# sail-sg/finetune-fair-diffusion

Measured on AMD Instinct MI355X. Metric: training-images/sec (SD-v1.5 512^2, 20-step DPM-Solver++ unroll, fairness-finetune step), higher is better.
Workload: dtype f16

## Files before the change

finetune_fair_diffusion_amd/ops.py:

```python
import ctypes
import os
import math

import torch

from . import lib as _lib

ACT = dict(none=0, silu=1, quick_gelu=2, gelu=3, relu=4, hardswish=5, hardsigmoid=6, geglu=7)
CONV_NORMAL, CONV_STRIDE2, CONV_UP2, CONV_TRANS2 = 0, 1, 2, 3
F16, F32 = _lib.torch_working_dtype(), torch.float32


def _stream():
    return ctypes.c_void_p(torch.cuda.current_stream().cuda_stream)


def _p(t):
    if t is None:
        return None
    assert t.is_cuda, "fairdiff ops need device tensors (no CPU path)"
    return ctypes.c_void_p(t.data_ptr())


DELAY = None
# ... 164 lines not shown
    d.alpha, d.M, d.N, d.K, d.batch = 1.0, rows, N, K, Z
    d.sA, d.sB, d.sC = a_view.stride(0), 0, rows * N
    _gemm_call(d, False)
    return out


def conv3x3(x, w, B, H, W, *, mode=CONV_NORMAL, bias=None, rowbias=None, residual=None, act="none", out=None, gn_stats=False):
    Cin = x.shape[1]
    Cout = w.shape[0]
    assert w.shape[1] == 9 * Cin and x.shape[0] == B * H * W
    _chk(x), _chk(w)
    if mode == CONV_NORMAL:
        Ho, Wo = H, W
    elif mode == CONV_STRIDE2:
        Ho, Wo = (H + 1) // 2, (W + 1) // 2
    else:
        Ho, Wo = 2 * H, 2 * W
    M = B * Ho * Wo
    if out is None:
        out = torch.empty((M, Cout), dtype=F16, device=x.device)
    d = _lib.GemmDesc()
    d.A, d.lda, d.B, d.ldb, d.C, d.ldc = x.data_ptr(), Cin, w.data_ptr(), 9 * Cin, out.data_ptr(), out.stride(0)
    if bias is not None:
        d.bias = _chk(bias, F32).data_ptr()
    if rowbias is not None:
        d.rowbias, d.ld_rowbias, d.rows_per_batch = _chk(rowbias).data_ptr(), rowbias.stride(0), (M if rowbias.shape[0] == 1 else Ho * Wo)
    if residual is not None:
        d.residual, d.ldr = _chk(residual).data_ptr(), residual.stride(0)
    d.alpha, d.M, d.N, d.K, d.act, d.batch = 1.0, M, Cout, 9 * Cin, ACT[act], 1
    d.out_dtype = 1 if out.dtype == F32 else 0
    d.conv, d.conv_mode, d.Bn, d.H, d.W, d.Cin, d.Ho, d.Wo = 1, mode, B, H, W, Cin, Ho, Wo
    _gemm_call(d, True, out, gn_stats)
    return out, Ho, Wo


CONV_UP2P, CONV_UP2P_BWD, CONV_UP2PI = 4, 5, 6
_BIG_TILES = (256320, 128320, 128160, 256128, 256256, 512128)
_NO_UP2P = os.environ.get("FD_NO_UP2P") is not None


def _up2p_desc(x, w, out, B, H, W, Cin, Cout, bwd, bias=None):
    d = _lib.GemmDesc()
    if bwd:
        d.K, d.conv_mode, d.H, d.W = 16 * Cin, CONV_UP2P_BWD, 2 * H, 2 * W
    else:
        d.K, d.conv_mode, d.H, d.W = 4 * Cin, CONV_UP2PI, H, W
    d.A, d.lda, d.B, d.ldb, d.C, d.ldc = x.data_ptr(), Cin, w.data_ptr(), d.K, out.data_ptr(), Cout
    if bias is not None:
        d.bias = _chk(bias, F32).data_ptr()
    d.alpha, d.M, d.N, d.act, d.batch, d.out_dtype = 1.0, B * H * W, Cout, ACT["none"], 1, 0
    d.conv, d.Bn, d.Cin, d.Ho, d.Wo = 1, B, Cin, H, W
    ws = gemm_workspace()
    d.workspace, d.workspace_bytes = ws.data_ptr(), ws.numel() * 4
    return d


def conv_up2(x, conv, B, H, W):
    Cin, Cout = conv.cin, conv.cout
    if not _NO_UP2P and Cin % 64 == 0 and Cout % 8 == 0:
        out = torch.empty((4 * B * H * W, Cout), dtype=F16, device=x.device)
        d = _up2p_desc(_chk(x), conv.wk_up2p, out, B, H, W, Cin, Cout, False, conv.bias)
        if _lib.get().fd_gemm_tile(ctypes.byref(d)) in _BIG_TILES:
            _gemm_call(d, True, out, gn_stats=(H * W) % 32 == 0)
            if getattr(out, "gn_stats", None) is not None:
                out.gn_stats = out.gn_stats + ((H * W) // 32,)
            return out, 2 * H, 2 * W
    return conv3x3(x, conv.wk, B, H, W, mode=CONV_UP2, bias=conv.bias)


def conv_up2_bwd(dy, conv, B, H, W):
    Cin, Cout = conv.cin, conv.cout
    if not _NO_UP2P and Cout % 64 == 0 and Cin % 8 == 0:
        out = torch.empty((B * H * W, Cin), dtype=F16, device=dy.device)
        d = _up2p_desc(_chk(dy), conv.wd_up2p, out, B, H, W, Cout, Cin, True)
        if _lib.get().fd_gemm_tile(ctypes.byref(d)) % 1000000 in _BIG_TILES:
            _gemm_call(d, True)
            return out
    dxu, _, _ = conv3x3(dy, conv.wd, B, 2 * H, 2 * W)
    return downsum2x2(dxu, B, H, W, Cin)


def conv_small_cin(x, w, bias, B, H, W, Cin, Cout, k, stride=1, nchw=True, act="none"):
    pad = (k - 1) // 2
    Ho, Wo = (H + 2 * pad - k) // stride + 1, (W + 2 * pad - k) // stride + 1
    y = torch.empty((B * Ho * Wo, Cout), dtype=F16, device=x.device)
    assert x.is_contiguous() and x.dtype in (F16, F32)
    _call("fd_conv_small_cin", _p(x), int(x.dtype == F32), int(nchw), _p(_chk(w, F32)), _p(bias), _p(y), B, H, W, Cin, Cout, k, stride,
          ACT[act], _stream())
    return y, Ho, Wo


def conv_small_cin_bwd(dy, w, B, H, W, Cin, Cout, k, stride=1, scale=1.0):
    dx = torch.empty((B, Cin, H, W), dtype=F32, device=dy.device)
    _call("fd_conv_small_cin_bwd", _p(_chk(dy)), _p(_chk(w, F32)), _p(dx), B, H, W, Cin, Cout, k, stride, scale, _stream())
    return dx


def nhwc_to_nchw(x, B, HW, C, *, out_dtype=F32, scale=1.0, lo=-math.inf, hi=math.inf):
    y = torch.empty((B, C, HW), dtype=out_dtype, device=x.device)
    _call("fd_nhwc_to_nchw", _p(x), x.stride(0), _p(y), int(out_dtype == F32), B, HW, C, scale, lo, hi, _stream())
    return y


def clamp_bwd(pre, dimg, B, HW, C, lo=-1.0, hi=1.0):
    out = torch.empty_like(dimg)
    _call("fd_clamp_bwd", _p(pre), pre.stride(0), _p(_chk(dimg, F32)), _p(out), B, HW, C, lo, hi, _stream())
    return out


_scratch = {}


def scratch(nfloats, device):
    key = (device.index if device.index is not None else torch.cuda.current_device(), torch.cuda.current_stream().cuda_stream)
    t = _scratch.get(key)
    if t is None or t.numel() < nfloats:
        t = torch.empty(max(nfloats, 1 << 22), dtype=F32, device=device)
        _scratch[key] = t
    return t


def groupnorm(x1, x2, B, HW, groups, eps, gamma, beta, silu):
    C1, C2 = x1.shape[1], (x2.shape[1] if x2 is not None else 0)
    st = torch.empty((B, groups, 2), dtype=F32, device=x1.device)
    y = torch.empty((B * HW, C1 + C2), dtype=F16, device=x1.device)
    s1, s2 = getattr(x1, "gn_stats", None), (getattr(x2, "gn_stats", None) if x2 is not None else None)
    if (s1 is not None and (x2 is None or s2 is not None) and HW % s1[1] == 0 and (s2 is None or HW % s2[1] == 0)
            and ((C1 + C2) // groups) % 10 == 0 and s1[0].shape[0] * s1[1] == B * HW and (s2 is None or s2[0].shape[0] * s2[1] == B * HW)):
        per1 = s1[2] if len(s1) > 2 else 0
        per2 = s2[2] if (s2 is not None and len(s2) > 2) else 0
        _call("fd_groupnorm_fwd_stats_p", _p(_chk(x1)), C1, _p(x2), C2, B, HW, groups, eps, _p(gamma), _p(beta), int(silu), _p(y), _p(st),
              _p(s1[0]), s1[1], per1, _p(s2[0]) if s2 is not None else None, s2[1] if s2 is not None else 0, per2, _stream())
        return y, st
    sc = scratch(B * 64 * groups * 2, x1.device)
    _call("fd_groupnorm_fwd", _p(_chk(x1)), C1, _p(x2), C2, B, HW, groups, eps, _p(gamma), _p(beta), int(silu), _p(y), _p(st), _p(sc), _stream())
    return y, st


def groupnorm_bwd(x1, x2, dy, B, HW, groups, stats, gamma, beta, silu, add1=None, add2=None, need_dx2=True):
    C1, C2 = x1.shape[1], (x2.shape[1] if x2 is not None else 0)
    dx1 = torch.empty_like(x1)
    dx2 = torch.empty_like(x2) if (x2 is not None and need_dx2) else None
    sc = scratch(B * 65 * groups * 2, x1.device)
    _call("fd_groupnorm_bwd", _p(x1), C1, _p(x2), C2, _p(_chk(dy)), B, HW, groups, _p(stats), _p(gamma), _p(beta), int(silu), _p(sc),
          _p(add1), _p(add2), _p(dx1), _p(dx2), _stream())
    return dx1, dx2


def geglu_bwd_interleaved(proj_il, dy):
    M, F2 = proj_il.shape
    d = torch.empty_like(proj_il)
    _call("fd_geglu_bwd_interleaved", _p(_chk(proj_il)), _p(_chk(dy)), _p(d), M, F2 // 2, _stream())
    return d


def layernorm(x, gamma, beta, eps=1e-5, save_stats=False):
    M, C = x.shape
    y = torch.empty_like(x)
    st = torch.empty((M, 2), dtype=F32, device=x.device) if save_stats else None
    _call("fd_layernorm_fwd", _p(_chk(x)), _p(gamma), _p(beta), _p(y), _p(st), M, C, eps, _stream())
    return (y, st) if save_stats else y


def layernorm_bwd(x, dy, gamma, stats, add=None):
    M, C = x.shape
    dx = torch.empty_like(x)
    _call("fd_layernorm_bwd", _p(_chk(x)), _p(_chk(dy)), _p(gamma), _p(stats), _p(add), _p(dx), M, C, _stream())
    return dx


def geglu(proj):
    M, F2 = proj.shape
    y = torch.empty((M, F2 // 2), dtype=F16, device=proj.device)
    _call("fd_geglu_fwd", _p(_chk(proj)), _p(y), M, F2 // 2, _stream())
    return y


def geglu_bwd(proj, dy):
    M, F2 = proj.shape
    d = torch.empty_like(proj)
    _call("fd_geglu_bwd", _p(proj), _p(_chk(dy)), _p(d), M, F2 // 2, _stream())
    return d


def act_fwd(x, act):
    y = torch.empty_like(x)
    _call("fd_act_fwd", _p(_chk(x)), _p(y), x.numel(), ACT[act], _stream())
    return y


def act_bwd(z, dy, act):
    dx = torch.empty_like(z)
    _call("fd_act_bwd", _p(_chk(z)), _p(_chk(dy)), _p(dx), z.numel(), ACT[act], _stream())
    return dx


def add(a, b, sa=1.0, sb=1.0, out=None):
    if out is None:
        out = torch.empty_like(a)
    _call("fd_add", _p(_chk(a)), _p(b), _p(out), a.numel(), sa, sb, _stream())
    return out


def copy_cols(src, dst, cols):
    _call("fd_copy_cols", _p(src), src.stride(0), _p(dst), dst.stride(0), src.shape[0], cols, _stream())


def _rows(t):
    assert t.dtype == F16 and t.dim() == 2 and t.stride(1) == 1, (t.dtype, t.shape, t.stride())
    return t.stride(0)


def transpose_btc(x, B, T, C, Tp=None, out=None):
    Tp = Tp or ((T + 7) // 8 * 8)
    y = torch.empty((B, C, Tp), dtype=F16, device=x.device) if out is None else out
    assert y.shape == (B, C, Tp) and y.dtype == F16 and y.is_contiguous()
    _call("fd_transpose_btc", _p(x), _rows(x), _p(y), B, T, C, Tp, _stream())
    return y


def downsum2x2(x, B, H, W, C):
    y = torch.empty((B * H * W, C), dtype=F16, device=x.device)
    _call("fd_downsum2x2", _p(_chk(x)), _p(y), B, H, W, C, _stream())
    return y


def softmax_rows(x, scale=1.0, mask=None, mask_t=0, mask_ht=0):
    rows, cols = x.numel() // x.shape[-1], x.shape[-1]
    y = torch.empty_like(x)
    _call("fd_softmax_rows", _p(_chk(x)), _p(y), rows, cols, scale, _p(mask), mask_t, mask_ht, _stream())
    return y


def softmax_rows_bwd(p, dp, scale=1.0):
    rows, cols = p.numel() // p.shape[-1], p.shape[-1]
    ds = torch.empty_like(p)
    _call("fd_softmax_rows_bwd", _p(_chk(p)), _p(_chk(dp)), _p(ds), rows, cols, scale, _stream())
    return ds


def to_f16(x, scale=1.0):
    y = torch.empty(x.shape, dtype=F16, device=x.device)
    _call("fd_cast_f32_to_f16", _p(_chk(x, F32)), _p(y), x.numel(), scale, _stream())
    return y


def to_f32(x, scale=1.0):
    y = torch.empty(x.shape, dtype=F32, device=x.device)
    _call("fd_cast_f16_to_f32", _p(_chk(x)), _p(y), x.numel(), scale, _stream())
    return y


LOG2E = 1.4426950408889634
PRESCALED_Q = os.environ.get("FD_NO_PRESCALED_Q") is None


def q_prescale(d):
    return (d ** -0.5) * LOG2E if (PRESCALED_Q and d % 16 == 8) else None


def attn_fwd(q, k, v, B, H, Tq, Tk, d, kv_div=1, scale=None, need_lse=False, kv_rows=None, prescaled=False):
    Tkr = kv_rows or Tk
    assert _rows(v) == _rows(k) and v.shape == k.shape
    o = torch.empty((q.shape[0], H * d), dtype=F16, device=q.device)
    lse = torch.empty((B, H, Tq), dtype=F32, device=q.device) if need_lse else None
    scale = scale if scale is not None else d ** -0.5
    _call("fd_attn_fwd", _p(q), _p(k), _p(v), _p(o), _p(lse), B, H, Tq, Tk, Tkr, d, kv_div,
          -scale if prescaled else scale, _rows(q), _rows(k), _stream())
    return (o, lse) if need_lse else o


def attn_bwd(q, k, v, o, do, lse, B, H, Tq, Tk, d, kv_div=1, scale=None, dk_acc=None, dv_acc=None, kv_rows=None, dqkv=None,
             dk_out=None, dv_out=None, prescaled=False):
    scale = scale if scale is not None else d ** -0.5
    if prescaled:
        scale = -scale
    Tkr = kv_rows or Tk
    C = H * d
    assert _rows(k) == _rows(v)
    Dd = torch.empty((B, H, Tq), dtype=F32, device=q.device)
    if dqkv is not None:
        assert kv_div == 1 and dqkv.shape == (q.shape[0], 3 * C) and dqkv.is_contiguous() and Tkr == Tk and dqkv.dtype == F16
        dq, dk, dv = dqkv[:, :C], dqkv[:, C:2 * C], dqkv[:, 2 * C:]
        lddkv = 3 * C
    else:
        dq = torch.empty((q.shape[0], C), dtype=F16, device=q.device)
        lddkv = C
        if dk_out is not None:
            assert dk_out.dtype == F32 and dv_out.dtype == F32 and dk_out.shape == (k.shape[0], C) and dv_out.shape == dk_out.shape and Tkr == Tk
            assert dk_out.is_contiguous() and dv_out.is_contiguous() and B % kv_div == 0
            slabs = torch.empty((2, kv_div) + tuple(dk_out.shape), dtype=F32, device=q.device)
            dk, dv = slabs[0], slabs[1]
        elif dk_acc is not None:
            dk, dv = dk_acc, dv_acc
            assert dk.dtype == F32 and dv.dtype == F32 and dk.shape == (k.shape[0], C) and Tkr == Tk
        else:
            assert kv_div == 1, "shared K/V (kv_div > 1) needs the fp32 accumulators dk_acc / dv_acc"
            mk = torch.empty if Tkr == Tk else torch.zeros
            dk, dv = mk((k.shape[0], C), dtype=F16, device=q.device), mk((k.shape[0], C), dtype=F16, device=q.device)
    _call("fd_attn_bwd_dq", _p(q), _p(k), _p(v), _p(_chk(do)), _p(lse), _p(Dd), _p(_chk(o)), _p(dq), B, H, Tq, Tk, Tkr, d,
          kv_div, scale, _rows(q), _rows(k), _rows(dq), _stream())
    _call("fd_attn_bwd_dkdv", _p(q), _p(k), _p(v), _p(do), _p(lse), _p(Dd), _p(dk), _p(dv), B, H, Tq, Tk, Tkr, d, kv_div, scale,
          _rows(q), _rows(k), lddkv, 2 if dk_out is not None else int(dk_acc is not None), _stream())
    if dk_out is not None:
        n = dk_out.numel()
        _call("fd_sum_slabs", _p(dk), _p(dk_out), kv_div, n, _stream())
# ... 259 lines not shown
```

finetune_fair_diffusion_amd/unet.py:

```python
import math

import torch

from . import ops
from .layers import (F16, F32, Conv3x3, Linear, LoRAPair, Norm, ParamBank, ResnetBlock, lora_linear_bwd, lora_linear_fwd)
from .weights import UNetConfig, unet_attn_names, unet_lora_param_shapes, unet_param_shapes


BWD_SLOT = [None]


class _Out:
    def __init__(self, sample):
        self.sample = sample


class LoRAAttnProcessor:

    def __init__(self, hidden_size, cross_attention_dim=None, rank=4):
        self.hidden_size, self.cross_attention_dim, self.rank = hidden_size, cross_attention_dim, rank

    def to(self, *a, **k):
        return self

# ... 1 lines not shown
class AttnLoRA:

    def __init__(self, bank, name):
        self.q, self.k, self.v, self.out = (LoRAPair(bank, f"{name}.{p}_lora.down.weight", f"{name}.{p}_lora.up.weight")
                                            for p in ("to_q", "to_k", "to_v", "to_out"))
        dev = bank.flat.device
        rp = self.q.rp
        if self.q.K == self.k.K:
            C = self.q.N
            self.down_qkv16 = torch.zeros((3 * rp, C), dtype=F16, device=dev)
            self.down_qkvT16 = torch.zeros((C, 3 * rp), dtype=F16, device=dev)
            self.up_qkv16 = torch.zeros((3 * C, 3 * rp), dtype=F16, device=dev)
            self.upT_qkv16 = torch.zeros((3 * rp, 3 * C), dtype=F16, device=dev)
            for i, p in enumerate((self.q, self.k, self.v)):
                p.place(self.down_qkv16[i * rp:(i + 1) * rp], self.down_qkvT16[:, i * rp:(i + 1) * rp],
                        self.up_qkv16[i * C:(i + 1) * C, i * rp:(i + 1) * rp], self.upT_qkv16[i * rp:(i + 1) * rp, i * C:(i + 1) * C])
            self.down_kv16 = self.down_qkv16[rp:]
        else:
            self.down_kv16 = torch.zeros((2 * rp, self.k.K), dtype=F16, device=dev)
            self.q.place()
            self.k.place(down16=self.down_kv16[:rp])
            self.v.place(down16=self.down_kv16[rp:])
        self.out.place()

    def pairs(self):
        return (self.q, self.k, self.v, self.out)

    def refresh(self):
        from .layers import refresh_pairs
        refresh_pairs(self.pairs())


class TransformerBlock:

    def __init__(self, sd, p, dev, C, heads, groups, xdim):
        self.C, self.heads, self.d, self.groups, self.xdim = C, heads, C // heads, groups, xdim
        self.p = p
        self.norm = Norm(sd, p + "norm", dev)
        self.proj_in = Linear(sd, p + "proj_in", dev, conv1x1=True)
        self.proj_out = Linear(sd, p + "proj_out", dev, conv1x1=True)
        b = p + "transformer_blocks.0."
        self.ln1, self.ln2, self.ln3 = Norm(sd, b + "norm1", dev), Norm(sd, b + "norm2", dev), Norm(sd, b + "norm3", dev)
        self.q1, self.k1, self.v1, self.o1 = (Linear(sd, b + "attn1." + n, dev) for n in ("to_q", "to_k", "to_v", "to_out.0"))
        assert self.q1.bias is None and self.k1.bias is None and self.v1.bias is None
        self.wqkv = torch.cat([self.q1.w, self.k1.w, self.v1.w], 0).contiguous()
        self._wqkvT = None
        self.q2, self.k2, self.v2, self.o2 = (Linear(sd, b + "attn2." + n, dev) for n in ("to_q", "to_k", "to_v", "to_out.0"))
        ff1, self.ff2 = Linear(sd, b + "ff.net.0.proj", dev), Linear(sd, b + "ff.net.2", dev)
        self.ff1_wi, self.ff1_bi = ops.interleave_geglu(ff1.w, ff1.bias)
        self._ff1_wiT = None
        self.lora1 = self.lora2 = None
        self.name1, self.name2 = b + "attn1.processor", b + "attn2.processor"
        self.cross = None
        self.lean = False

    def prepare_cross(self, enc, Bk, L, record, static=False):
        lo = self.lora2
        te = ops.gemm(enc, lo.down_kv16) if lo is not None else None
        rp = lo.k.rp if lo is not None else 0
        old = None
        if lo is not None:
            K = ops.gemm(enc, self.k2.w, a2=te[:, :rp], b2=lo.k.up16)
            V = ops.gemm(enc, self.v2.w, a2=te[:, rp:], b2=lo.v.up16)
        elif static:
            old = self.cross if (self.cross is not None and self.cross.get("static") and self.cross["K"].shape == (Bk * L, self.C)) else None
            K = ops.gemm(enc, self.k2.w, out=old["K"] if old else None)
            V = ops.gemm(enc, self.v2.w, out=old["V"] if old else None)
            if old is None:
                self.static_generation = getattr(self, "static_generation", 0) + 1
        else:
            K, V = ops.gemm(enc, self.k2.w), ops.gemm(enc, self.v2.w)
        self.cross = dict(static=bool(static and lo is None), K=K, V=V, Bk=Bk, L=L, enc=enc, te=te)
        if ops.FUSED_CROSS and L <= ops.CROSS_LP and self.C in ops.CROSS_WIDTHS and self.heads == 8:
            self.cross["Vt80"] = ops.transpose_btc(V, Bk, L, self.C, ops.CROSS_LP, out=old.get("Vt80") if (static and old) else None)
        if record:
            self.cross["dK"] = torch.zeros((Bk * L, self.C), dtype=F32, device=enc.device)
            self.cross["dV"] = torch.zeros((Bk * L, self.C), dtype=F32, device=enc.device)

    def finish_cross_backward(self, gscale, need_denc):
        c, lo = self.cross, self.lora2
        if c.get("slots") is not None:
            c["dK"] += c["slots"][:, 0].sum(dim=0)
            c["dV"] += c["slots"][:, 1].sum(dim=0)
            c["slots"] = None
        dK, dV = ops.to_f16(c["dK"]), ops.to_f16(c["dV"])
        rp = lo.k.rp if lo is not None else 0
        te = c["te"]
        denc = lora_linear_bwd(dK, c["enc"], te[:, :rp] if te is not None else None, self.k2, lo.k if lo else None, gscale, need_dx=need_denc)
        denc = lora_linear_bwd(dV, c["enc"], te[:, rp:] if te is not None else None, self.v2, lo.v if lo else None, gscale, residual=denc,
                               need_dx=need_denc)
        return denc

    def forward(self, x, B, H, W, ctx=None, pair=False):
        HW, C, h, d = H * W, self.C, self.heads, self.d
        rec = ctx is not None
        g, st = ops.groupnorm(x, None, B, HW, self.groups, 1e-6, self.norm.gamma, self.norm.beta, False)
        h0, n1, ln1 = ops.gemm(g, self.proj_in.w, bias=self.proj_in.bias, ln=(self.ln1.gamma, self.ln1.beta, 1e-5))
        l1 = self.lora1
        qs = ops.q_prescale(d)
        csq = (qs, C) if qs is not None else None
        if l1 is not None:
            t1 = ops.gemm(n1, l1.down_qkv16)
            qkv = ops.gemm(n1, self.wqkv, a2=t1, b2=l1.up_qkv16, colscale=csq)
        else:
            t1 = None
            qkv = ops.gemm(n1, self.wqkv, colscale=csq)
        q, k, v = qkv[:, :C], qkv[:, C:2 * C], qkv[:, 2 * C:]
        o, lse = ops.attn_fwd(q, k, v, B, h, HW, HW, d, 1, need_lse=True, prescaled=qs is not None)
        l2 = self.lora2
        cr = self.cross
        if (not pair and cr.get("Vt80") is not None and self.q2.bias is None and self.o2.bias is not None and (ops.FUSED_CROSS_TRAIN or (not rec and l2 is None))
                and ops.cross_block_ok(B * HW, C, h, cr["L"], HW, l2.q.rp if l2 is not None else 0)):
            h1, to1 = lora_linear_fwd(o, self.o1, l1.out if l1 else None, residual=h0)
            qs2 = ops.q_prescale(d)
            h2, n3, ln3, r = ops.cross_attn_block(h1, (self.ln2.gamma, self.ln2.beta, 1e-5), self.q2.w, cr["K"], cr["Vt80"], cr["L"], self.o2.w, self.o2.bias,
                                                  (self.ln3.gamma, self.ln3.beta, 1e-5), h, HW, B // cr["Bk"], lora_q=l2.q if l2 else None,
                                                  lora_o=l2.out if l2 else None, record=rec, q_prescaled=qs2 is not None)
            lean = rec and self.lean
            proj = torch.empty((n3.shape[0], self.ff1_wi.shape[0]), dtype=F16, device=n3.device) if rec and not lean else None
            gg = ops.gemm(n3, self.ff1_wi, bias=self.ff1_bi, act="geglu", aux=proj)
            h3 = ops.gemm(gg, self.ff2.w, bias=self.ff2.bias, residual=h2)
            out = ops.gemm(h3, self.proj_out.w, bias=self.proj_out.bias, residual=x, gn_stats=True)
            if rec:
                ctx.append(dict(x=x, st=st, h0=h0, ln1=ln1, n1=None if lean else n1, t1=t1, qkv=qkv, o=o, lse=lse, to1=to1, h1=h1, ln2=r["ln2"], n2=None if lean else r["n2"], tq2=r["tq2"], q2=r["q2"],
                                o2=r["o2"], lse2=r["lse2"], to2=r["to2"], h2=h2, ln3=ln3, proj=proj, pair=False, qs=qs is not None, qs2=qs2 is not None))
            return out
        (h1, n2, ln2), to1 = lora_linear_fwd(o, self.o1, l1.out if l1 else None, residual=h0, ln=(self.ln2.gamma, self.ln2.beta, 1e-5))
        qs2 = ops.q_prescale(d)
        q2, tq2 = lora_linear_fwd(n2, self.q2, l2.q if l2 else None, colscale=(qs2, C) if qs2 is not None else None)
        B2 = 2 * B if pair else B
        q2f, h1f, xf = (torch.cat([q2, q2]), torch.cat([h1, h1]), torch.cat([x, x])) if pair else (q2, h1, x)
        kv_div = B2 // cr["Bk"]
        o2, lse2 = ops.attn_fwd(q2f, cr["K"], cr["V"], B2, h, HW, cr["L"], d, kv_div, need_lse=True, prescaled=qs2 is not None)
        (h2, n3, ln3), to2 = lora_linear_fwd(o2, self.o2, l2.out if l2 else None, residual=h1f, ln=(self.ln3.gamma, self.ln3.beta, 1e-5))
        lean = rec and self.lean
        proj = torch.empty((n3.shape[0], self.ff1_wi.shape[0]), dtype=F16, device=n3.device) if rec and not lean else None
        gg = ops.gemm(n3, self.ff1_wi, bias=self.ff1_bi, act="geglu", aux=proj)
        h3 = ops.gemm(gg, self.ff2.w, bias=self.ff2.bias, residual=h2)
        out = ops.gemm(h3, self.proj_out.w, bias=self.proj_out.bias, residual=xf, gn_stats=True)
        if rec:
            ctx.append(dict(x=x, st=st, h0=h0, ln1=ln1, n1=None if lean else n1, t1=t1, qkv=qkv, o=o, lse=lse, to1=to1, h1=h1, ln2=ln2, n2=None if lean else n2,
                            tq2=tq2, q2=q2f, o2=o2, lse2=lse2, to2=to2, h2=h2, ln3=ln3, proj=proj, pair=pair, qs=qs is not None, qs2=qs2 is not None))
        return out

    def backward(self, d_out, B, H, W, c, gscale, need_dx=True):
        with ops.wgrad_batch():
            return self._backward(d_out, B, H, W, c, gscale, need_dx)

    def _backward(self, d_out, B, H, W, c, gscale, need_dx=True):
        HW, C, h, d = H * W, self.C, self.heads, self.d
        l1, l2 = self.lora1, self.lora2
        pair = c.get("pair", False)
        dh3 = ops.gemm(d_out, self.proj_out.wT)
        dgg = ops.gemm(dh3, self.ff2.wT)
        proj = c["proj"]
        if proj is None:
            proj = ops.gemm(ops.layernorm(c["h2"], self.ln3.gamma, self.ln3.beta, 1e-5), self.ff1_wi, bias=self.ff1_bi)
        dproj = ops.geglu_bwd_interleaved(proj, dgg)
        del proj
        if self._ff1_wiT is None:
            self._ff1_wiT = self.ff1_wi.t().contiguous()
        dn3 = ops.gemm(dproj, self._ff1_wiT)
        dh2 = ops.layernorm_bwd(c["h2"], dn3, self.ln3.gamma, c["ln3"], add=dh3)
        do2 = lora_linear_bwd(dh2, c["o2"], c["to2"], self.o2, l2.out if l2 else None, gscale)
        cr = self.cross
        kv_div = B // cr["Bk"]
        slot = BWD_SLOT[0] if cr.get("slots") is not None else None
        if slot is not None:
            dq2, _, _ = ops.attn_bwd(c["q2"], cr["K"], cr["V"], c["o2"], do2, c["lse2"], B, h, HW, cr["L"], d, kv_div,
                                     dk_out=cr["slots"][slot, 0], dv_out=cr["slots"][slot, 1], prescaled=c.get("qs2", False))
        else:
            dq2, _, _ = ops.attn_bwd(c["q2"], cr["K"], cr["V"], c["o2"], do2, c["lse2"], B, h, HW, cr["L"], d, kv_div,
                                     dk_acc=cr["dK"], dv_acc=cr["dV"], prescaled=c.get("qs2", False))
        if pair:
            B = B // 2
            M = B * HW
            dq2 = ops.add(dq2[:M], dq2[M:])
            dh2 = ops.add(dh2[:M], dh2[M:])
            if need_dx:
                d_out = ops.add(d_out[:M], d_out[M:])
        n2 = c["n2"] if (c["n2"] is not None or l2 is None) else ops.layernorm(c["h1"], self.ln2.gamma, self.ln2.beta, 1e-5)
        dn2 = lora_linear_bwd(dq2, n2, c["tq2"], self.q2, l2.q if l2 else None, gscale)
        dh1 = ops.layernorm_bwd(c["h1"], dn2, self.ln2.gamma, c["ln2"], add=dh2)
        do1 = lora_linear_bwd(dh1, c["o"], c["to1"], self.o1, l1.out if l1 else None, gscale)
        qkv = c["qkv"]
        dqkv = torch.empty_like(qkv)
        ops.attn_bwd(qkv[:, :C], qkv[:, C:2 * C], qkv[:, 2 * C:], c["o"], do1, c["lse"], B, h, HW, HW, d, 1, dqkv=dqkv, prescaled=c.get("qs", False))
        if self._wqkvT is None:
            self._wqkvT = self.wqkv.t().contiguous()
        if l1 is not None:
            t1, rp = c["t1"], l1.q.rp
            n1 = c["n1"] if c["n1"] is not None else ops.layernorm(c["h0"], self.ln1.gamma, self.ln1.beta, 1e-5)
            u = ops.gemm(dqkv, l1.upT_qkv16)
            for i, pair in enumerate((l1.q, l1.k, l1.v)):
                gd, gu = pair.grads()
                ops.lora_wgrad(dqkv[:, i * C:(i + 1) * C], t1[:, i * rp:(i + 1) * rp], gu, pair.r, 1, pair.r, scale=1.0 / gscale)
                ops.lora_wgrad(n1, u[:, i * rp:(i + 1) * rp], gd, 1, pair.K, pair.r, scale=1.0 / gscale)
            dn1 = ops.gemm(dqkv, self._wqkvT, a2=u, b2=l1.down_qkvT16) if need_dx else None
        else:
            dn1 = ops.gemm(dqkv, self._wqkvT) if need_dx else None
        if not need_dx:
            return None
        dh0 = ops.layernorm_bwd(c["h0"], dn1, self.ln1.gamma, c["ln1"], add=dh1)
        dg = ops.gemm(dh0, self.proj_in.wT)
        dx, _ = ops.groupnorm_bwd(c["x"], None, dg, B, HW, self.groups, c["st"], self.norm.gamma, self.norm.beta, False, add1=d_out)
        return dx


class UNet2DConditionModel:
    def __init__(self, cfg: UNetConfig, state_dict, device):
        self.config, self.device = cfg, device
        shapes = unet_param_shapes(cfg)
        missing = [k for k in shapes if k not in state_dict]
        if missing:
            raise KeyError(f"UNet state_dict is missing {len(missing)} tensors, e.g. {missing[:3]}")
        sd, dev = state_dict, device
        boc, g, heads, xdim, n = cfg.block_out_channels, cfg.norm_num_groups, cfg.attention_head_dim, cfg.cross_attention_dim, cfg.layers_per_block
        self.temb_dim = boc[0] * 4
        w = sd["conv_in.weight"].to(dev, F32)
        self.conv_in_w = w.permute(2, 3, 1, 0).reshape(9 * cfg.in_channels, boc[0]).contiguous()
        self.conv_in_b = sd["conv_in.bias"].to(dev, F32).contiguous()
        self.time1, self.time2 = Linear(sd, "time_embedding.linear_1", dev), Linear(sd, "time_embedding.linear_2", dev)
        self.resnets, self.transformers = [], []

        def res(p):
            r = ResnetBlock(sd, p, dev, g, 1e-5)
            self.resnets.append(r)
            return r

        def tr(p, c):
            t = TransformerBlock(sd, p, dev, c, heads, g, xdim)
            self.transformers.append(t)
            return t

        self.down = []
        cout = boc[0]
        for i, t in enumerate(cfg.down_block_types):
            cout = boc[i]
            blk = dict(res=[res(f"down_blocks.{i}.resnets.{j}.") for j in range(n)],
                       attn=[tr(f"down_blocks.{i}.attentions.{j}.", cout) for j in range(n)] if t.startswith("CrossAttn") else None,
                       down=Conv3x3(sd, f"down_blocks.{i}.downsamplers.0.conv", dev) if i != len(boc) - 1 else None)
            self.down.append(blk)
        c = boc[-1]
        self.mid = dict(res=[res("mid_block.resnets.0."), res("mid_block.resnets.1.")], attn=[tr("mid_block.attentions.0.", c)])
        self.up = []
        rev = list(reversed(boc))
        for i, t in enumerate(cfg.up_block_types):
            cout = rev[i]
            blk = dict(res=[res(f"up_blocks.{i}.resnets.{j}.") for j in range(n + 1)],
                       attn=[tr(f"up_blocks.{i}.attentions.{j}.", cout) for j in range(n + 1)] if t.startswith("CrossAttn") else None,
                       up=Conv3x3(sd, f"up_blocks.{i}.upsamplers.0.conv", dev) if i != len(boc) - 1 else None)
            self.up.append(blk)
        self.norm_out = Norm(sd, "conv_norm_out", dev)
        self.conv_out = Conv3x3(sd, "conv_out", dev)
        wo = sd["conv_out.weight"].to(dev, F32)
        self.conv_out_wd = wo.flip(2, 3).permute(2, 3, 0, 1).reshape(9 * cfg.out_channels, boc[0]).contiguous()
        ws, bs, off = [], [], 0
        for r in self.resnets:
            ws.append(r.temb_w.to(dev, F16))
            bs.append(r.temb_b.to(dev, F32))
            r.temb_slice = (off, off + ws[-1].shape[0])
            off += ws[-1].shape[0]
        self.temb_proj_w = torch.cat(ws, 0).contiguous()
        self.temb_proj_b = torch.cat(bs, 0).contiguous()
        self.lora_bank = None
        self._tr_by_name = {}
        for t in self.transformers:
            self._tr_by_name[t.name1] = (t, 1)
            self._tr_by_name[t.name2] = (t, 2)
        self.temb_table = None
        self._ctx = None

    @property
    def attn_processors(self):
        return {n: (getattr(self._tr_by_name[n][0], f"lora{self._tr_by_name[n][1]}")) for n in unet_attn_names(self.config)}

    def set_attn_processor(self, processors):
        names = unet_attn_names(self.config)
        if set(processors) != set(names):
            raise ValueError(f"expected {len(names)} attention processors, got {len(processors)} with different names")
        ranks = {p.rank for p in processors.values()}
        if len(ranks) != 1:
            raise ValueError(f"all LoRA processors must share one rank, got {sorted(ranks)}")
        shapes = unet_lora_param_shapes(self.config, ranks.pop())
        for n, p in processors.items():
            cin = shapes[n + ".to_k_lora.down.weight"][1]
            hid = shapes[n + ".to_q_lora.down.weight"][1]
            if p.hidden_size != hid or (p.cross_attention_dim or hid) != cin:
                raise ValueError(f"{n}: processor sizes ({p.hidden_size}, {p.cross_attention_dim}) do not match the U-Net ({hid}, {cin})")
        return self.add_lora(next(iter(processors.values())).rank, seed=getattr(next(iter(processors.values())), "seed", 0))

    @property
    def dtype(self):
        return F16

    def to(self, *a, **k):
        return self

    def enable_gradient_checkpointing(self):
        return None

    def train(self, mode=True):
        return self

    def eval(self):
        return self

    def requires_grad_(self, flag=False):
        return self

    def add_lora(self, rank, state_dict=None, seed=0):
        shapes = unet_lora_param_shapes(self.config, rank)
        self.lora_bank = ParamBank(shapes, self.device)
        if state_dict is None:
            from .weights import synthetic_state_dict
            state_dict = synthetic_state_dict(shapes, seed=seed)
# ... 211 lines not shown
```

include/fairdiff_hip.h:

```cpp
#ifndef FAIRDIFF_HIP_H
#define FAIRDIFF_HIP_H
#include <stdint.h>
#ifdef __cplusplus
extern "C" {
#endif

#define FD_OK 0
#define FD_ERR_ARG (-1)
#define FD_ERR_LAUNCH (-2)
#define FD_ABI_VERSION 4

enum { FD_ACT_NONE = 0, FD_ACT_SILU = 1, FD_ACT_QUICK_GELU = 2, FD_ACT_GELU = 3, FD_ACT_RELU = 4,
       FD_ACT_HARDSWISH = 5, FD_ACT_HARDSIGMOID = 6,
       FD_ACT_GEGLU = 7 };
enum { FD_OUT_F16 = 0, FD_OUT_F32 = 1 };
enum { FD_CONV_NORMAL = 0, FD_CONV_STRIDE2 = 1, FD_CONV_UP2 = 2, FD_CONV_TRANS2 = 3,
       FD_CONV_UP2P = 4,
       FD_CONV_UP2P_BWD = 5,
       FD_CONV_UP2PI = 6 };

const char* fd_last_error(void);
int fd_version(void);
const char* fd_working_dtype(void);
const char* fd_build_info(void);

typedef struct fd_gemm_desc {
    int32_t struct_size;
    const void* A;  int64_t lda;
    const void* B;  int64_t ldb;
    const void* A2; int64_t lda2;
    const void* B2; int64_t ldb2;
    void* C;        int64_t ldc;
    const float* bias;
    const void* rowbias; int64_t ld_rowbias; int32_t rows_per_batch;
    const void* residual; int64_t ldr;
    float alpha;
    int32_t M, N, K, K2;
    int32_t act, out_dtype;
    int32_t batch; int64_t sA, sB, sC, sR;
    int32_t conv, conv_mode, Bn, H, W, Cin, Ho, Wo;
    void* workspace; int64_t workspace_bytes;
    float* gn_stats;
    float colscale; int32_t colscale_cols;
} fd_gemm_desc;
int fd_gemm(const fd_gemm_desc* d, void* stream);
int fd_gemm_stats_rows(const fd_gemm_desc* d);
int fd_gemm_tile(const fd_gemm_desc* d);
int fd_gemm_kernel_name(const fd_gemm_desc* d, char* buf, int n);

int fd_conv_small_cin(const void* x, int x_is_f32, int nchw, const float* w, const float* bias, void* y,
                      int B, int H, int W, int Cin, int Cout, int ksize, int stride, int act, void* stream);
int fd_nhwc_to_nchw(const void* x, int64_t ldx, void* y, int y_is_f32, int B, int HW, int C, float scale, float lo, float hi, void* stream);
int fd_clamp_bwd(const void* pre, int64_t ldx, const float* dimg, float* dpre, int B, int HW, int C, float lo, float hi, void* stream);

int fd_groupnorm_fwd(const void* x1, int C1, const void* x2, int C2, int B, int HW, int groups, float eps, const float* gamma,
                     const float* beta, int silu, void* y, float* mean_rstd, float* scratch, void* stream);
int fd_groupnorm_fwd_stats(const void* x1, int C1, const void* x2, int C2, int B, int HW, int groups, float eps, const float* gamma,
                           const float* beta, int silu, void* y, float* mean_rstd, const float* st1, int rows1, const float* st2, int rows2,
                           void* stream);
int fd_groupnorm_fwd_stats_p(const void* x1, int C1, const void* x2, int C2, int B, int HW, int groups, float eps, const float* gamma,
                             const float* beta, int silu, void* y, float* mean_rstd, const float* st1, int rows1, int per1, const float* st2,
                             int rows2, int per2, void* stream);
int fd_groupnorm_bwd(const void* x1, int C1, const void* x2, int C2, const void* dy, int B, int HW, int groups,
                     const float* mean_rstd, const float* gamma, const float* beta, int silu,
                     float* scratch, const void* add1, const void* add2, void* dx1, void* dx2, void* stream);

int fd_layernorm_fwd(const void* x, const float* gamma, const float* beta, void* y, float* mean_rstd ,
                     int M, int C, float eps, void* stream);
int fd_layernorm_bwd(const void* x, const void* dy, const float* gamma, const float* mean_rstd, const void* add ,
                     void* dx, int M, int C, void* stream);

int fd_geglu_fwd(const void* proj , void* y , int M, int F, void* stream);
int fd_geglu_bwd(const void* proj, const void* dy, void* dproj, int M, int F, void* stream);
int fd_geglu_bwd_interleaved(const void* proj, const void* dy, void* dproj, int M, int F, void* stream);
int fd_act_fwd(const void* x, void* y, int64_t n, int act, void* stream);
int fd_act_bwd(const void* z, const void* dy, void* dx, int64_t n, int act, void* stream);
int fd_add(const void* a, const void* b, void* y, int64_t n, float sa, float sb, void* stream);
int fd_copy_cols(const void* src, int64_t lds, void* dst, int64_t ldd, int64_t M, int cols, void* stream);
int fd_transpose_btc(const void* x , int64_t ldx, void* y , int B, int T, int C, int Tp, void* stream);
int fd_downsum2x2(const void* x , void* y , int B, int H, int W, int C, void* stream);
int fd_softmax_rows(const void* x, void* y, int64_t rows, int cols, float scale, const float* mask, int mask_t, int mask_ht, void* stream);
int fd_softmax_rows_bwd(const void* p, const void* dp, void* ds, int64_t rows, int cols, float scale, void* stream);
int fd_cast_f32_to_f16(const float* x, void* y, int64_t n, float scale, void* stream);
int fd_cast_f16_to_f32(const void* x, float* y, int64_t n, float scale, void* stream);

int fd_attn_fwd(const void* q, const void* k, const void* v, void* o, float* lse, int B, int H, int Tq, int Tk,
                int Tkr, int d, int kv_div, float scale, int ldq, int ldk, void* stream);
int fd_attn_bwd_prep(const void* o, const void* d_o, float* D, int B, int H, int T, int d, void* stream);
int fd_attn_bwd_dq(const void* q, const void* k, const void* v, const void* d_o, const float* lse,
                   float* D, const void* o, void* dq, int B, int H, int Tq, int Tk, int Tkr, int d, int kv_div, float scale,
                   int ldq, int ldkv, int lddq, void* stream);
int fd_attn_bwd_dkdv(const void* q, const void* k, const void* v, const void* d_o,
                     const float* lse, const float* D, void* dk, void* dv, int B, int H, int Tq, int Tk, int Tkr, int d,
                     int kv_div, float scale, int ldq, int ldkv, int lddkv, int accumulate, void* stream);
int fd_sum_slabs(const float* in, float* out, int nslab, int64_t n, void* stream);

typedef struct fd_cross_block_desc {
    int32_t struct_size;
    const void* x;
    const float* ln2_gamma; const float* ln2_beta; float ln2_eps;
    const void* wq;
    const void* k; const void* vt; int32_t L, Lp;
    const void* wo; const float* bo;
    const float* ln3_gamma; const float* ln3_beta; float ln3_eps;
    void* y; void* yn; float* yn_stats;
    int32_t M, C, heads, rows_per_sample, kv_div;
    float scale;
    const void* lora_q_down; int64_t ld_q_down; const void* lora_q_up; int64_t ld_q_up;
    const void* lora_o_down; int64_t ld_o_down; const void* lora_o_up; int64_t ld_o_up;
    int32_t lora_rp;
    void* n2_out; float* ln2_stats; void* q_out; void* tq_out; void* o_out; float* lse_out; void* to_out;
    int32_t q_prescaled;
} fd_cross_block_desc;
int fd_cross_attn_block(const fd_cross_block_desc* d, void* stream);

int fd_small_attn_fwd(const void* q, const void* k, const void* v, void* o, float* P, const int32_t* key_valid, int B, int H, int T,
                      int d, float scale, int causal, void* stream);
int fd_small_attn_bwd(const void* q, const void* k, const void* v, const float* P, const void* d_o, void* dq, void* dk, void* dv,
                      int B, int H, int T, int d, float scale, void* stream);

int fd_lora_wgrad(const void* X, int64_t ldx, const void* T, int64_t ldt, float* G, int64_t g_stride_n, int64_t g_stride_r,
                  int M, int N, int R, float scale, float* scratch, int64_t scratch_elems, void* stream);

#define FD_WGRAD_MAX 16
typedef struct fd_wgrad_desc {
    int32_t struct_size;
    const void* X; int64_t ldx;
    const void* T; int64_t ldt;
    float* G; int64_t g_stride_n, g_stride_r;
    int32_t M, N, R;
    float scale;
} fd_wgrad_desc;
int fd_lora_wgrad_multi(const fd_wgrad_desc* descs, int n, float* scratch, int64_t scratch_elems, void* stream);

typedef struct fd_lora_refresh_desc {
    int32_t struct_size;
    const float* down; const float* up;
    void* d16; int64_t ld_d16;
    void* dT16; int64_t ld_dT16;
    void* u16; int64_t ld_u16;
    void* uT16; int64_t ld_uT16;
    int32_t r, rp, K, N;
    float scale;
} fd_lora_refresh_desc;
int fd_lora_refresh_multi(const fd_lora_refresh_desc* descs, int n, void* stream);

int fd_cfg_dpm_step(const float* eps, float guidance, float* lat, const float* x0_prev, float* x0_out,
                    float alpha_t, float sigma_t, float c_x, float c_d0, float c_d1, int64_t n, void* stream);

int fd_grad_finite_scale(float* g, int64_t n, float scale, int32_t* nonfinite_flag, void* stream);
int fd_adamw_ema(float* p, const float* g, float* m, float* v, float* ema, int64_t n, float lr, float beta1, float beta2,
                 float eps, float weight_decay, int32_t step, float ema_one_minus_decay, void* stream);

int fd_dwconv_fwd(const void* x, const float* w , const float* bias, void* y, int B, int H, int W, int C,
                  int k, int stride, int act, void* stream);
int fd_dwconv_bwd(const void* dy, const float* w, void* dx, int B, int H, int W, int C, int k, int stride, void* stream);
int fd_avgpool_hw(const void* x, void* y, int B, int HW, int C, void* stream);
int fd_avgpool_hw_bwd(const void* dy , const void* add , void* dx, int B, int HW, int C, void* stream);
int fd_scale_channels(const void* x, const void* s, void* y, int B, int HW, int C, void* stream);
int fd_scale_channels_bwd(const void* x, const void* s, const void* dy, void* dx, void* ds , int B, int HW, int C, void* stream);
int fd_conv_small_cin_bwd(const void* dy , const float* w, float* dx ,
                          int B, int H, int W, int Cin, int Cout, int ksize, int stride, float scale, void* stream);
int fd_crop_resize_fwd(const void* img, const int32_t* boxes, float fill, void* chips, int B, int H, int W, int S, void* stream);
int fd_crop_resize_bwd(const float* dchips , const int32_t* boxes, float* dimg ,
                       int B, int H, int W, int S, void* stream);

int fd_patchify_fwd(const void* chips, void* patches, const float* mean3, const float* std3, int N, int S, int P, int Kp, void* stream);
int fd_patchify_bwd(const void* dpatches, float* dchips, const float* std3, int N, int S, int P, int Kp, float scale, int accumulate,
                    void* stream);
int fd_warp_affine_fwd(const void* img, const int32_t* src_index, const float* A, float fill, void* chips, int n_chips, int H, int W,
                       int S, void* stream);
int fd_warp_affine_bwd(const float* dchips, const int32_t* src_index, const float* A, float* dimg, int n_chips, int B, int H, int W,
                       int S, void* stream);
int fd_rect_scale(float* dimg, const int32_t* rects, const float* factors, int B, int H, int W, void* stream);

int fd_ot_assign_sum(const double* cost, const int32_t* counts, float* plan, int32_t* seats, int N, int K, int S, void* stream);
int fd_ot_expected_targets(const double* cost, const int32_t* counts, const double* weights, int32_t* seats, int32_t* targets, double* uncertainty,
                           int N, int K, int S, void* stream);

#define FD_EVAL_MAX_ATTR 3
#define FD_EVAL_MAX_K 4
#define FD_EVAL_COUNTS 32
#define FD_EVAL_ATTR_STRIDE 6
#define FD_EVAL_OFF_P1_HI 18
#define FD_EVAL_OFF_P1_LO 19
#define FD_EVAL_OFF_P1_MID 20
#define FD_EVAL_OFF_JOINT 21
#define FD_EVAL_OFF_JOINT_VALID 29
#define FD_EVAL_PALETTE 6
int fd_eval_tally(const float* probs, int N, int ld, const int32_t* attr_c0, const int32_t* attr_k, int n_attr, int32_t* counts, void* stream);
int fd_eval_grid_u8(const void* images, const int32_t* order, const int32_t* boxes, const int32_t* preds, const float* maxprob, const uint8_t* palette,
                    uint8_t* grid, int N, int H, int W, int rows, int cols, void* stream);

#ifdef __cplusplus
}
#endif
#endif
```

Before: 6.249.

## Fuse feed-forward backward GEMM, GEGLU grad, and second GEMM into one kernel

Adds a HIP kernel that computes the FF2 transpose GEMM, the GEGLU backward gate and the FF1 transpose GEMM in one pass for C=320 transformer blocks. The intermediate dgg and dproj tensors stay in LDS and registers instead of round-tripping through HBM. A LayerNorm-backward epilogue exists but is off by default, so layernorm_bwd still runs as a separate launch. Other widths fall back to the old four-launch path. The fused kernel uses a single grid of M/128 blocks with a large LDS footprint, which may lower occupancy compared with the tuned standalone GEMMs.

```diff
diff --git a/finetune_fair_diffusion_amd/csrc/ff_bwd.hip b/finetune_fair_diffusion_amd/csrc/ff_bwd.hip
--- /dev/null
+++ b/finetune_fair_diffusion_amd/csrc/ff_bwd.hip
@@ -0,0 +1,235 @@
+#include "gemm_device.h"
+
+struct FfBwdArgs {
+    const f16* dh3;
+    const f16* w2t;
+    const f16* proj;
+    const f16* w1t;
+    const f16* h2;
+    const float* gamma;
+    const float* mean_rstd;
+    f16* dh2;
+    f16* dn3;
+    int M, C;
+};
+
+constexpr int FFB_BM = 128, FFB_NC = 32;
+template <int C_>
+constexpr size_t ffb_lds_bytes() {
+    return (size_t)(2 * C_ * 64 + 2 * (C_ / 64) * FFB_NC * 64 + 2 * FFB_BM * 64) * sizeof(f16);
+}
+
+template <int C_>
+__global__ __launch_bounds__(512) void ff_bwd_kernel(FfBwdArgs a) {
+    constexpr int BM = FFB_BM, NC = FFB_NC, NW = 8;
+    constexpr int KT1 = C_ / 64;
+    constexpr int KQ = C_ / 32;
+    constexpr int K2 = 8 * C_;
+    constexpr int NCH = 4 * C_ / NC;
+    constexpr int G1 = C_ / 8, G1I = G1 / NW;
+    constexpr int G2 = KT1 * (NC / 8), G2I = (G2 + NW - 1) / NW;
+    constexpr int TM = 4, TN = C_ / 4 / 16;
+    static_assert(C_ % 64 == 0 && G1 % NW == 0 && (C_ / 4) % 16 == 0 && NC == 32, "tile geometry");
+    extern __shared__ __attribute__((aligned(16))) f16 smem[];
+    f16* W1s = smem;
+    f16* W2s = W1s + 2 * C_ * 64;
+    f16* A2s = W2s + 2 * KT1 * NC * 64;
+
+    const int tid = threadIdx.x, lane = tid & 63, wave = tid >> 6;
+    const int l15 = lane & 15, lg = lane >> 4;
+    const int wm = wave >> 2, wn = wave & 3;
+    const int lrow = lane >> 3;
+    const int kchunk = ((lane & 7) ^ lrow) * 8;
+    const int fsw = l15 & 7;
+    const int m0 = blockIdx.x * BM;
+    const int mrow = m0 + wave * 16 + l15;
+
+    auto issue_w1 = [&](int c, int buf) {
+#pragma unroll
+        for (int i = 0; i < G1I; ++i) {
+            const int g = wave + i * NW;
+            glds16(a.w1t + (int64_t)(g * 8 + lrow) * K2 + c * 64 + kchunk, W1s + (buf * C_ + g * 8) * 64);
+        }
+    };
+    auto issue_w2 = [&](int c, int buf) {
+#pragma unroll
+        for (int i = 0; i < G2I; ++i) {
+            const int g = wave + i * NW;
+            if (g < G2) {
+                const int kt = g / (NC / 8), r8 = g % (NC / 8);
+                glds16(a.w2t + (int64_t)(c * NC + r8 * 8 + lrow) * C_ + kt * 64 + kchunk, W2s + ((buf * KT1 + kt) * NC + r8 * 8) * 64);
+            }
+        }
+    };
+    const f16* prow = a.proj + (int64_t)mrow * K2 + lg * 8;
+    auto load_proj = [&](int c, f16x8 (&pr)[2]) {
+#pragma unroll
+        for (int j = 0; j < 2; ++j) pr[j] = *(const f16x8*)(prow + c * (2 * NC) + j * 32);
+    };
+
+    issue_w2(0, 0);
+    issue_w1(0, 0);
+    issue_w2(1, 1);
+    f16x8 af[KQ];
+#pragma unroll
+    for (int q = 0; q < KQ; ++q) af[q] = *(const f16x8*)(a.dh3 + (int64_t)mrow * C_ + q * 32 + lg * 8);
+    f16x8 pcur[2], pnext[2];
+    load_proj(0, pcur);
+    load_proj(1, pnext);
+
+    f32x4 acc2[TM][TN];
+#pragma unroll
+    for (int i = 0; i < TM; ++i)
+#pragma unroll
+        for (int j = 0; j < TN; ++j) acc2[i][j] = (f32x4){0.f, 0.f, 0.f, 0.f};
+
+    auto stage1_gate = [&](int buf, const f16x8 (&pr)[2]) {
+        f32x4 acc1[2] = {{0.f, 0.f, 0.f, 0.f}, {0.f, 0.f, 0.f, 0.f}};
+        const f16* Bb = W2s + (buf * KT1 * NC + l15) * 64;
+#pragma unroll
+        for (int q = 0; q < KQ; ++q) {
+            const int slot = (((q & 1) * 4 + lg) ^ fsw) * 8;
+#pragma unroll
+            for (int j = 0; j < 2; ++j) {
+                const f16x8 bf = *(const f16x8*)(Bb + ((q >> 1) * NC + j * 16) * 64 + slot);
+                acc1[j] = FD_MFMA_16x16x32(bf, af[q], acc1[j]);
+            }
+        }
+#pragma unroll
+        for (int j = 0; j < 2; ++j) {
+            const f16x4 d = {(f16)acc1[j][0], (f16)acc1[j][1], (f16)acc1[j][2], (f16)acc1[j][3]};
+            f16x8 o;
+#pragma unroll
+            for (int r = 0; r < 4; ++r) {
+                const float av = (float)pr[j][2 * r], g = (float)pr[j][2 * r + 1], dj = (float)d[r];
+                float h = 0.5f * dj;
+                asm("" : "+v"(h));
+                h *= g;
+                asm("" : "+v"(h));
+                float ad = av * dj;
+                asm("" : "+v"(ad));
+                o[2 * r] = (f16)(h * (1.f + erf_as(g * 0.70710678118654752f)));
+                o[2 * r + 1] = (f16)(ad * gelu_erf_grad_f(g));
+            }
+            *(f16x8*)(A2s + (buf * BM + wave * 16 + l15) * 64 + ((j * 4 + lg) ^ fsw) * 8) = o;
+        }
+    };
+    auto stage2 = [&](int buf) {
+        const f16* Ab = A2s + (buf * BM + wm * 64 + l15) * 64;
+        const f16* Bb = W1s + (buf * C_ + wn * (TN * 16) + l15) * 64;
+#pragma unroll
+        for (int ks = 0; ks < 2; ++ks) {
+            const int slot = ((ks * 4 + lg) ^ fsw) * 8;
+            f16x8 fa[TM];
+#pragma unroll
+            for (int i = 0; i < TM; ++i) fa[i] = *(const f16x8*)(Ab + i * 16 * 64 + slot);
+#pragma unroll
+            for (int j = 0; j < TN; ++j) {
+                const f16x8 bf = *(const f16x8*)(Bb + j * 16 * 64 + slot);
+#pragma unroll
+                for (int i = 0; i < TM; ++i) acc2[i][j] = FD_MFMA_16x16x32(bf, fa[i], acc2[i][j]);
+            }
+        }
+    };
+
+    asm volatile("s_waitcnt vmcnt(0)" ::: "memory");
+    __syncthreads();
+    stage1_gate(0, pcur);
+#pragma unroll
+    for (int j = 0; j < 2; ++j) pcur[j] = pnext[j];
+
+#pragma unroll 1
+    for (int c = 0; c < NCH - 1; ++c) {
+        const int buf = c & 1;
+        asm volatile("s_waitcnt vmcnt(0)" ::: "memory");
+        __syncthreads();
+        issue_w1(c + 1, buf ^ 1);
+        issue_w2(min(c + 2, NCH - 1), buf);
+        load_proj(min(c + 2, NCH - 1), pnext);
+        stage1_gate(buf ^ 1, pcur);
+        stage2(buf);
+#pragma unroll
+        for (int j = 0; j < 2; ++j) pcur[j] = pnext[j];
+    }
+    asm volatile("s_waitcnt vmcnt(0)" ::: "memory");
+    __syncthreads();
+    stage2((NCH - 1) & 1);
+    __syncthreads();
+
+    constexpr int LDW = C_ + 8;
+    static_assert((size_t)BM * LDW * sizeof(f16) <= ffb_lds_bytes<C_>(), "LayerNorm staging does not fit");
+    f16* st = smem;
+#pragma unroll
+    for (int i = 0; i < TM; ++i)
+#pragma unroll
+        for (int j = 0; j < TN; ++j) {
+            const f32x4 v = acc2[i][j];
+            *(f16x4*)(st + (wm * 64 + i * 16 + l15) * LDW + wn * (TN * 16) + j * 16 + lg * 4) = (f16x4){(f16)v[0], (f16)v[1], (f16)v[2], (f16)v[3]};
+        }
+    __syncthreads();
+    if (a.dn3) {
+        if (lane < C_ / 8)
+#pragma unroll
+            for (int r = 0; r < 16; ++r)
+                *(f16x8*)(a.dn3 + (int64_t)(m0 + wave * 16 + r) * C_ + lane * 8) = *(const f16x8*)(st + (wave * 16 + r) * LDW + lane * 8);
+        return;
+    }
+
+    const int C = a.C;
+    float Cf = (float)C;
+    asm volatile("" : "+v"(Cf));
+    const int V = C >> 3;
+    const int v = lane;
+    float gm[8];
+#pragma unroll
+    for (int j = 0; j < 8; ++j) gm[j] = v < V ? a.gamma[v * 8 + j] : 0.f;
+#pragma unroll 1
+    for (int pass = 0; pass < 4; ++pass) {
+        const int lr0 = wave * 16 + pass * 4;
+        f16x8 xv[4], dv[4];
+#pragma unroll
+        for (int r = 0; r < 4; ++r)
+            if (v < V) {
+                xv[r] = *(const f16x8*)(a.h2 + (int64_t)(m0 + lr0 + r) * C + v * 8);
+                dv[r] = *(const f16x8*)(st + (lr0 + r) * LDW + v * 8);
+            }
+#pragma unroll
+        for (int r = 0; r < 4; ++r) {
+            const int row = m0 + lr0 + r;
+            float s0 = 0.f, s1 = 0.f;
+            const float mean = a.mean_rstd[row * 2], rstd = a.mean_rstd[row * 2 + 1];
+            if (v < V) {
+#pragma unroll
+                for (int j = 0; j < 8; ++j) {
+                    const float t = (float)dv[r][j] * gm[j];
+                    s0 += t;
+                    s1 += t * ((float)xv[r][j] - mean) * rstd;
+                }
+            }
+            const float m1 = wave_sum(s0) / Cf, m2 = wave_sum(s1) / Cf;
+            if (v < V) {
+                const f16x8 av = *(const f16x8*)(a.dh3 + (int64_t)row * C + v * 8);
+                f16x8 o;
+#pragma unroll
+                for (int j = 0; j < 8; ++j) {
+                    const float xh = ((float)xv[r][j] - mean) * rstd;
+                    const float t = (float)dv[r][j] * gm[j];
+                    o[j] = (f16)(rstd * (t - m1 - xh * m2) + (float)av[j]);
+                }
+                *(f16x8*)(a.dh2 + (int64_t)row * C + v * 8) = o;
+            }
+        }
+    }
+}
+
+extern "C" int fd_ff_bwd(const void* dh3, const void* ff2_wT, const void* proj, const void* ff1_wiT, const void* h2, const float* gamma,
+                         const float* mean_rstd, void* dh2, void* dn3, int M, int C, void* stream) {
+    FD_REQUIRE(C == 320 && M > 0 && M % FFB_BM == 0, "fd_ff_bwd: C=%d M=%d: needs C == 320 and M a positive multiple of %d", C, M, FFB_BM);
+    FD_REQUIRE(dh3 && ff2_wT && proj && ff1_wiT && (dn3 || (h2 && gamma && mean_rstd && dh2)), "fd_ff_bwd: null operand");
+    FfBwdArgs a{(const f16*)dh3, (const f16*)ff2_wT, (const f16*)proj, (const f16*)ff1_wiT, (const f16*)h2, gamma, mean_rstd, (f16*)dh2, (f16*)dn3, M, C};
+    constexpr size_t lds = ffb_lds_bytes<320>();
+    static std::once_flag once;
+    std::call_once(once, [] { (void)hipFuncSetAttribute((const void*)ff_bwd_kernel<320>, hipFuncAttributeMaxDynamicSharedMemorySize, (int)lds); });
+    hipLaunchKernelGGL(ff_bwd_kernel<320>, dim3(M / FFB_BM), dim3(512), lds, (hipStream_t)stream, a);
+    return fd_check_launch("fd_ff_bwd");
+}
diff --git a/finetune_fair_diffusion_amd/ops.py b/finetune_fair_diffusion_amd/ops.py
--- a/finetune_fair_diffusion_amd/ops.py
+++ b/finetune_fair_diffusion_amd/ops.py
@@ -340,6 +340,29 @@
     d = torch.empty_like(proj_il)
     _call("fd_geglu_bwd_interleaved", _p(_chk(proj_il)), _p(_chk(dy)), _p(d), M, F2 // 2, _stream())
     return d
+
+
+FUSED_FF_BWD = os.environ.get("FD_NO_FUSED_FF_BWD") is None
+FUSED_FF_BWD_LN = os.environ.get("FD_FUSED_FF_BWD_LN") is not None
+FF_BWD_WIDTHS = (320,)
+FF_BWD_ROWS = 128
+
+
+def ff_bwd_ok(M, C):
+    return FUSED_FF_BWD and C in FF_BWD_WIDTHS and M >= FF_BWD_ROWS and M % FF_BWD_ROWS == 0
+
+
+def ff_bwd(dh3, ff2_wT, proj_il, ff1_wiT, h2, gamma, stats, fuse_ln=None):
+    M, C = dh3.shape
+    if not ff_bwd_ok(M, C):
+        return layernorm_bwd(h2, gemm(geglu_bwd_interleaved(proj_il, gemm(dh3, ff2_wT)), ff1_wiT), gamma, stats, add=dh3)
+    assert ff2_wT.shape == (4 * C, C) and proj_il.shape == (M, 8 * C) and ff1_wiT.shape == (C, 8 * C) and h2.shape == (M, C) and stats.shape == (M, 2)
+    out = torch.empty_like(dh3)
+    if FUSED_FF_BWD_LN if fuse_ln is None else fuse_ln:
+        _call("fd_ff_bwd", _p(_chk(dh3)), _p(_chk(ff2_wT)), _p(_chk(proj_il)), _p(_chk(ff1_wiT)), _p(_chk(h2)), _p(gamma), _p(stats), _p(out), None, M, C, _stream())
+        return out
+    _call("fd_ff_bwd", _p(_chk(dh3)), _p(_chk(ff2_wT)), _p(_chk(proj_il)), _p(_chk(ff1_wiT)), None, None, None, None, _p(out), M, C, _stream())
+    return layernorm_bwd(h2, out, gamma, stats, add=dh3)
 
 
 def layernorm(x, gamma, beta, eps=1e-5, save_stats=False):
diff --git a/finetune_fair_diffusion_amd/unet.py b/finetune_fair_diffusion_amd/unet.py
--- a/finetune_fair_diffusion_amd/unet.py
+++ b/finetune_fair_diffusion_amd/unet.py
@@ -177,16 +177,13 @@
         l1, l2 = self.lora1, self.lora2
         pair = c.get("pair", False)
         dh3 = ops.gemm(d_out, self.proj_out.wT)
-        dgg = ops.gemm(dh3, self.ff2.wT)
         proj = c["proj"]
         if proj is None:
             proj = ops.gemm(ops.layernorm(c["h2"], self.ln3.gamma, self.ln3.beta, 1e-5), self.ff1_wi, bias=self.ff1_bi)
-        dproj = ops.geglu_bwd_interleaved(proj, dgg)
-        del proj
         if self._ff1_wiT is None:
             self._ff1_wiT = self.ff1_wi.t().contiguous()
-        dn3 = ops.gemm(dproj, self._ff1_wiT)
-        dh2 = ops.layernorm_bwd(c["h2"], dn3, self.ln3.gamma, c["ln3"], add=dh3)
+        dh2 = ops.ff_bwd(dh3, self.ff2.wT, proj, self._ff1_wiT, c["h2"], self.ln3.gamma, c["ln3"])
+        del proj
         do2 = lora_linear_bwd(dh2, c["o2"], c["to2"], self.o2, l2.out if l2 else None, gscale)
         cr = self.cross
         kv_div = B // cr["Bk"]
diff --git a/include/fairdiff_hip.h b/include/fairdiff_hip.h
--- a/include/fairdiff_hip.h
+++ b/include/fairdiff_hip.h
@@ -70,6 +70,9 @@
 int fd_layernorm_bwd(const void* x, const void* dy, const float* gamma, const float* mean_rstd, const void* add ,
                      void* dx, int M, int C, void* stream);
 
+int fd_ff_bwd(const void* dh3 , const void* ff2_wT , const void* proj , const void* ff1_wiT ,
+              const void* h2 , const float* gamma, const float* mean_rstd , void* dh2 , void* dn3 , int M, int C, void* stream);
+
 int fd_geglu_fwd(const void* proj , void* y , int M, int F, void* stream);
 int fd_geglu_bwd(const void* proj, const void* dy, void* dproj, int M, int F, void* stream);
 int fd_geglu_bwd_interleaved(const void* proj, const void* dy, void* dproj, int M, int F, void* stream);
diff --git a/scratch/mb_ff_bwd.py b/scratch/mb_ff_bwd.py
--- /dev/null
+++ b/scratch/mb_ff_bwd.py
@@ -0,0 +1,48 @@
+import sys, os, torch
+sys.path.insert(0, os.path.dirname(os.path.dirname(os.path.abspath(__file__))))
+from finetune_fair_diffusion_amd import ops
+dev = torch.device("cuda:0")
+def timeit(fn, n=20, rep=5):
+    for _ in range(3): fn()
+    ts = []
+    for _ in range(rep):
+        a, b = torch.cuda.Event(enable_timing=True), torch.cuda.Event(enable_timing=True)
+        a.record()
+        for _ in range(n): fn()
+        b.record(); torch.cuda.synchronize()
+        ts.append(a.elapsed_time(b) * 1000 / n)
+    return sorted(ts)[len(ts) // 2]
+for M, C in [(65536, 320), (32768, 320)]:
+    POOL = 3
+    h = lambda *s, sc=1.0: (torch.randn(*s, device=dev) * sc).to(ops.F16)
+    dh3 = [h(M, C) for _ in range(POOL)]; pr = [h(M, 8 * C) for _ in range(POOL)]; h2 = [h(M, C) for _ in range(POOL)]
+    w2t, w1t = h(4 * C, C, sc=C ** -0.5), h(C, 8 * C, sc=(8 * C) ** -0.5)
+    gamma, beta = torch.ones(C, device=dev), torch.zeros(C, device=dev)
+    st = [ops.layernorm(x, gamma, beta, 1e-5, save_stats=True)[1] for x in h2]
+    i = [0]
+    def nxt():
+        i[0] = (i[0] + 1) % POOL
+        return i[0]
+    def four():
+        k = nxt()
+        return ops.layernorm_bwd(h2[k], ops.gemm(ops.geglu_bwd_interleaved(pr[k], ops.gemm(dh3[k], w2t)), w1t), gamma, st[k], add=dh3[k])
+    def fused_ln():
+        k = nxt()
+        return ops.ff_bwd(dh3[k], w2t, pr[k], w1t, h2[k], gamma, st[k], fuse_ln=True)
+    def fused():
+        k = nxt()
+        return ops.ff_bwd(dh3[k], w2t, pr[k], w1t, h2[k], gamma, st[k], fuse_ln=False)
+    def parts():
+        k = nxt()
+        dgg = ops.gemm(dh3[k], w2t)
+        t1 = timeit(lambda: ops.gemm(dh3[nxt()], w2t))
+        t2 = timeit(lambda: ops.geglu_bwd_interleaved(pr[nxt()], dgg))
+        dp = ops.geglu_bwd_interleaved(pr[k], dgg)
+        t3 = timeit(lambda: ops.gemm(dp, w1t))
+        dn3 = ops.gemm(dp, w1t)
+        t4 = timeit(lambda: ops.layernorm_bwd(h2[nxt()], dn3, gamma, st[k], add=dh3[k]))
+        return t1, t2, t3, t4
+    assert ops.ff_bwd_ok(M, C)
+    print(f"M={M} C={C}: four launches {timeit(four):.1f} us   ff_bwd + layernorm_bwd {timeit(fused):.1f} us   ff_bwd with LayerNorm epilogue {timeit(fused_ln):.1f} us"
+          f"   (parts: gemm {parts()})", flush=True)
+    del dh3, pr, h2
```

Result: slower. 6.155 (-1.5%).
